# AIM-Harvard/pyradiomics

Hardware: AMD Instinct MI355X
Metric: Mvoxels/s for GLCM+GLRLM build, 512^3 vol @32 bins (higher is better)
Workload: dtype u8 levels / u32 counts / f64 out; 1 GPU; GLCM+GLRLM matrix build, 512^3 int32+uint8 volume resident in HBM, 32 grey levels, full mask, 13 angles, uniform levels; one volume per GPU (batch sharding, no collective); size=512, levels=32, dist=uniform, deferred_mode=pipeline

## Files before the change

### pyradiomics_amd/csrc/kernels_sweep.h

```cpp
#pragma once
#include "prad_runtime.h"

namespace prad {

typedef unsigned int u32;
typedef unsigned long long u64;

__global__ void __launch_bounds__(256) pack_levels_kernel(const int *__restrict__ image,
                                                          const uint8_t *__restrict__ mask, long long n, int NX,
                                                          int pitch, int padw, int Ng,
                                                          uint8_t *__restrict__ levels, int *__restrict__ flags,
                                                          int vec_ok, int shift, uint8_t *__restrict__ rowzero = nullptr) {
  const long long tid = (long long)blockIdx.x * blockDim.x + threadIdx.x;
  const long long nthreads = (long long)gridDim.x * blockDim.x;
  const bool linear = (padw == 0 && pitch == NX);
  int bad = 0;
  long long done = 0;
  if (vec_ok) {
    const long long n16 = n >> 4;
    const int upr = NX >> 4;
    const int4 *im4 = reinterpret_cast<const int4 *>(image);
    const uint4 *mk4 = reinterpret_cast<const uint4 *>(mask);
    for (long long t = tid; t < n16; t += nthreads) {
      const uint4 m = mk4[t];
// ... 323 lines not shown
__device__ __forceinline__ bool steps_break_group(W (&w)[LPL], const unsigned (&v)[U], const int (&sb)[U],
                                                  const bool (&uw)[U], int lane4) {
  bool m = false;
#pragma unroll
  for (int k = 0; k < U; k++) {
#pragma unroll
    for (int j = 0; j < LPL; j++) {
      const bool brk = uw[k] || (sb[k] == lane4 + j);
      m |= w[j].template step_brk<CHECK>((int)((v[k] >> (8 * j)) & 0xffu), brk);
    }
  }
  return m;
}
template <bool DO_GLCM, bool DO_GLRLM, bool FUSED>
__device__ __forceinline__ void flush_block_hist(const u32 *lds, const HistLayout &h, int Nr, int slot,
                                                 u32 *__restrict__ glcm_acc, u32 *__restrict__ glrlm_acc) {
  __syncthreads();
  const int Ng = h.Ng;
  if (FUSED) {
    const int Q = Ng + 1, P = (h.RS + 1) * Q;
    u32 *gd = glcm_acc + (size_t)slot * Ng * Ng;
    for (int i = threadIdx.x; i < Ng * Ng; i += blockDim.x) {
      const int p = i / Ng, c = i - p * Ng;
      if (p == c) continue;
      u32 v = 0;
      for (int l = 0; l <= h.RS; l++) v += lds[(p + 1) * P + l * Q + c + 1];
      if (v) atomicAdd(gd + i, v);
    }
    u32 *rd = glrlm_acc + (size_t)slot * Ng * Nr;
    for (int i = threadIdx.x; i < Ng * h.RS; i += blockDim.x) {
      const int p = i / h.RS, l = i - p * h.RS;
      u32 v = 0;
      for (int c = 0; c <= Ng; c++) v += lds[(p + 1) * P + l * Q + c];
      if (v) atomicAdd(rd + (size_t)p * Nr + l, v);
    }
    for (int i = threadIdx.x; i < Ng * h.RL; i += blockDim.x) {
      const int p = i / h.RL, l = h.RS + (i - p * h.RL);
      const u32 v = lds[h.g0 + i];
      if (v && l < Nr) atomicAdd(rd + (size_t)p * Nr + l, v);
    }
    return;
  }
  if (DO_GLCM) {
    u32 *dst = glcm_acc + (size_t)slot * Ng * Ng;
    for (int i = threadIdx.x; i < Ng * Ng; i += blockDim.x) {
      const u32 v = lds[i];
      if (v) atomicAdd(dst + i, v);
    }
  }
  if (DO_GLRLM) {
    const u32 *hr = lds + h.glrlm0;
    u32 *dst = glrlm_acc + (size_t)slot * Ng * Nr;
    for (int i = threadIdx.x; i < h.RS * Ng; i += blockDim.x) {
      const u32 v = hr[i];
      if (v) atomicAdd(dst + (size_t)(i % Ng) * Nr + (i / Ng), v);
// ... 279 lines not shown
    pairs += (unsigned long long)r * v;
    found |= (r > 0 && v != 0);
  }
  const u32 *grow = glcm_acc + ((size_t)a * Ng + i) * Ng;
  for (int j = lane; j < Ng; j += 64) found |= (grow[j] != 0);
  for (int o = 32; o > 0; o >>= 1) pairs += __shfl_xor(pairs, o);
  if (lane == 0) glcm_out[((size_t)i * Ng + i) * Na + a] = (double)pairs;
  if (__ballot(found) != 0 && lane == 0) multi[a] = 1;
}

struct AngleSet {
  int count;
  int off[PRAD_MAX_SWEEP][3];
};
template <typename T>
__global__ void __launch_bounds__(256) multi_check_kernel(AngleSet A, const T *__restrict__ L, int Nz, int Ny,
                                                          int Nx, int pitch, int *__restrict__ multi) {
  const int a = blockIdx.y;
  if (multi[a]) return;
  const int dz = A.off[a][0], dy = A.off[a][1], dx = A.off[a][2];
  const long long n = (long long)Nz * Ny * Nx, plane = (long long)Ny * Nx;
  const long long stride = (long long)gridDim.x * blockDim.x;
  for (long long i = (long long)blockIdx.x * blockDim.x + threadIdx.x; i < n; i += stride) {
    int z = (int)(i / plane);
    const int r = (int)(i - (long long)z * plane);
    int y = r / Nx, x = r - y * Nx;
    const int pz = z - dz, py = y - dy, px = x - dx;
    if ((unsigned)pz < (unsigned)Nz && (unsigned)py < (unsigned)Ny && (unsigned)px < (unsigned)Nx) continue;
    int cnt = 0;
    while ((unsigned)z < (unsigned)Nz && (unsigned)y < (unsigned)Ny && (unsigned)x < (unsigned)Nx) {
      cnt += L[((long long)z * Ny + y) * pitch + x] != 0;
      if (cnt > 1) {
        multi[a] = 1;
        return;
      }
      z += dz; y += dy; x += dx;
    }
  }
}

__global__ void finalize_glcm_kernel(const u32 *__restrict__ acc, const u32 *__restrict__ glrlm_acc, int Ng, int Nr,
                                     int Na, int diag_from_runs, double *__restrict__ out) {
  const long long idx = (long long)blockIdx.x * blockDim.x + threadIdx.x;
  const long long total = (long long)Ng * Ng * Na;
  if (idx >= total) return;
  const int a = (int)(idx % Na);
  const long long ij = idx / Na;
  const int i = (int)(ij / Ng), j = (int)(ij - (long long)i * Ng);
  if (diag_from_runs && i == j) return;
  out[idx] = (double)acc[(size_t)a * Ng * Ng + ij];
}

__global__ void __launch_bounds__(256) finalize_glcm_diag_kernel(const u32 *__restrict__ glcm_acc, u32 *glrlm_acc, int Ng, int Nr,
// ... 57 lines not shown
```

### pyradiomics_amd/csrc/kernels_sweepfw.h

```cpp
#pragma once
#include "kernels_sweep.h"

namespace prad {

enum FwPhase { FP_INIT, FP_GRAB, FP_CTRL, FP_ISSUE, FP_WAIT_ROWS, FP_WAIT_PACK, FP_GROUP, FP_PACK, FP_SLOW, FP_FLUSH, FP_DRAIN,
               FP_TOTAL, FP_REALTIME, FP_NGROUP, FP_NGROUP_PACK, FP_NSLOW, FP_COUNT };
#ifdef PRAD_FW_STAMPS
__device__ unsigned long long prad_fw_stamps[2 * 8192 * FP_COUNT];
struct FwClock {
  unsigned long long last, first, rt0;
  unsigned acc[FP_COUNT];
  __device__ __forceinline__ void start() {
#pragma unroll
    for (int i = 0; i < FP_COUNT; i++) acc[i] = 0;
    rt0 = __builtin_amdgcn_s_memrealtime();
    first = last = __builtin_readcyclecounter();
  }
  template <int PH>
  __device__ __forceinline__ void lap() {
    const unsigned long long now = __builtin_readcyclecounter();
    acc[PH] += (unsigned)(now - last);
    last = now;
  }
  template <int PH>
// ... 779 lines not shown
    asm volatile("" : "+v"(z));
    asm volatile(PRAD_FW_RCOL(0) PRAD_FW_RCOL(1) PRAD_FW_RCOL(2) PRAD_FW_RCOL(3)
                 : [s] "+v"(s), [t] "=&v"(t)
                 : [c] "v"(c), [x] "v"(x), [one] "v"(one), [P4] "s"(T.P4), [Q] "s"(T.Q), [z] "v"(z)
                 : "vcc", "memory");
  } else {
    asm volatile(PRAD_FW_RCOL_NZ(0) PRAD_FW_RCOL_NZ(1) PRAD_FW_RCOL_NZ(2) PRAD_FW_RCOL_NZ(3)
                 : [s] "+v"(s), [t] "=&v"(t)
                 : [c] "v"(c), [x] "v"(x), [one] "v"(one), [P4] "s"(T.P4), [Q] "s"(T.Q)
                 : "vcc", "memory");
  }
#undef PRAD_FW_RCOL
#undef PRAD_FW_RCOL_NZ
}

template <bool LONG, bool ZA>
__device__ __forceinline__ void fw_rows_role(const HistLayout &h, const FwTab &T, u32 *lds, const uint8_t *__restrict__ L,
                                             long long nrows, int NX, int pitch, int bx, int nblocks) {
  const int lane = threadIdx.x & 63, wave = threadIdx.x >> 6, wpb = blockDim.x >> 6;
  const int dummy = T.dummy0b + 4 * lane;
  u32 one = 1;
  asm volatile("" : "+v"(one));
  uint8_t *tile = reinterpret_cast<uint8_t *>(lds) + ((fw_lds_bytes(h) + 15) & ~(size_t)15) + (size_t)wave * 64 * PRAD_ROW_PITCH;
  const int RSTEP = nrows >= 4096 ? 8 : 1;
  const long long ngroups = RSTEP == 8 ? ((nrows + 511) / 512) * 8 : (nrows + 63) / 64;
  const long long nwaves = (long long)nblocks * wpb;
  const bool vec16 = (pitch & 15) == 0 && ((uintptr_t)L & 15) == 0;
  for (long long grp = (long long)bx * wpb + wave; grp < ngroups; grp += nwaves) {
    const long long r0 = RSTEP == 8 ? (grp >> 3) * 512 + (grp & 7) : grp * 64;
    int s = 0;
    u32 pw = 0;
    uint4 nx4[4];
    auto fetch = [&](int xc) __attribute__((always_inline)) {
#pragma unroll
      for (int j = 0; j < 4; j++) {
        const int rr = j * 16 + (lane >> 2);
        const int cx = xc + (lane & 3) * 16;
        uint4 q = make_uint4(0, 0, 0, 0);
        if (r0 + RSTEP * rr < nrows && cx < NX) {
          q = *reinterpret_cast<const uint4 *>(L + (r0 + RSTEP * rr) * pitch + cx);
          const int valid = NX - cx;
          if (valid < 16) {
            u32 *qw = reinterpret_cast<u32 *>(&q);
#pragma unroll
            for (int wd = 0; wd < 4; wd++) {
              const int keep = valid - 4 * wd;
// ... 14 lines not shown
      } else {
        const bool xin = xc + lane < NX;
#pragma unroll 8
        for (int rr = 0; rr < 64; rr++) {
          uint8_t b = 0;
          if (xin && r0 + RSTEP * rr < nrows) b = L[(r0 + RSTEP * rr) * pitch + xc + lane];
          tile[rr * PRAD_ROW_PITCH + lane] = b;
        }
      }
      __builtin_amdgcn_wave_barrier();
      const uint4 *row = reinterpret_cast<const uint4 *>(tile + lane * PRAD_ROW_PITCH);
#pragma unroll
      for (int q = 0; q < 4; q++) {
        const uint4 d = row[q];
        const u32 wds[4] = {d.x, d.y, d.z, d.w};
        const unsigned m = (pw >> 24) ? (unsigned)(s - __mul24((int)(pw >> 24), T.P4)) : 0u;
        if (LONG && __ballot(m + 16 * T.Q > (unsigned)T.lenlim) != 0) {
#pragma unroll 1
          for (int k = 0; k < 4; k++) {
            const u32 c = wds[k], x = __builtin_amdgcn_alignbyte(c, pw, 3);
            const unsigned m4 = (pw >> 24) ? (unsigned)(s - __mul24((int)(pw >> 24), T.P4)) : 0u;
            if (__ballot(m4 + 4 * T.Q > (unsigned)T.lenlim) != 0) {
#pragma unroll
              for (int b = 0; b < 4; b++) fw_checked<LONG>(T, dummy, s, (int)((x >> (8 * b)) & 0xffu), (int)((c >> (8 * b)) & 0xffu), false);
            } else {
              fw_row_word<ZA>(T, one, s, c, x);
            }
            pw = c;
          }
        } else {
#pragma unroll
          for (int k = 0; k < 4; k++) {
            fw_row_word<ZA>(T, one, s, wds[k], __builtin_amdgcn_alignbyte(wds[k], pw, 3));
            pw = wds[k];
          }
        }
      }
      __builtin_amdgcn_wave_barrier();
    }
    fw_checked<LONG>(T, dummy, s, (int)(pw >> 24), 0, false);
  }
}

template <bool LONG>
__global__ void __launch_bounds__(1024) sweep_fw_rows_kernel(const uint8_t *__restrict__ L, long long nrows, int NX, int pitch,
                                                            int slot, int Ng, int Nr, int RS, u32 *__restrict__ glcm_acc,
                                                            u32 *__restrict__ glrlm_acc, int *__restrict__ flags) {
  extern __shared__ u32 lds[];
  if (flags[0]) return;
  const HistLayout h = hist_layout(true, true, true, Ng, RS);
  if ((unsigned)(size_t)((lds_u32 *)lds) != 0u) {
    if (threadIdx.x == 0) atomicExch(flags + 2, 1);
    return;
  }
  for (int i = threadIdx.x; i < h.words + Ng + 1; i += blockDim.x) lds[i] = 0;
  __syncthreads();
  FwTab T;
  T.init(h, Nr, glrlm_acc + (size_t)slot * Ng * Nr);
  if (flags[3] != 0) fw_rows_role<LONG, true>(h, T, lds, L, nrows, NX, pitch, (int)blockIdx.x, (int)gridDim.x);
  else fw_rows_role<LONG, false>(h, T, lds, L, nrows, NX, pitch, (int)blockIdx.x, (int)gridDim.x);
  flush_block_hist<true, true, true>(lds + Ng + 1, h, Nr, slot, glcm_acc, glrlm_acc);
}

template <bool LONG, int K, bool HASPAD, bool PACK>
__global__ void __launch_bounds__(1024) sweep_fw_kernel(FwSet set, PackJob pj, const uint8_t *__restrict__ L,
                                                        const uint8_t *__restrict__ rowzero, int Ng, int Nr, int RS,
                                                        u32 *__restrict__ glcm_acc, u32 *__restrict__ glrlm_acc,
                                                        int *__restrict__ work, int *__restrict__ flags) {
  extern __shared__ u32 lds[];
  int role = 0;
  while (role + 1 < set.count && (int)blockIdx.x >= set.first_block[role + 1]) role++;
  const int bx = (int)blockIdx.x - set.first_block[role], nblocks = set.first_block[role + 1] - set.first_block[role];
  const int wpb = (int)(blockDim.x >> 6);
  const long long pw = __builtin_amdgcn_readfirstlane((int)(blockIdx.x * wpb + (threadIdx.x >> 6)));
  PackWave pk(pj, pw, (long long)gridDim.x * wpb);
  FwClock clk;
  clk.start();
#ifdef PRAD_FW_SETPRIO
  __builtin_amdgcn_s_setprio(PRAD_FW_SETPRIO);
#endif
  if (flags[0] == 0) {
    const bool anyzero = flags[3] != 0;
    const HistLayout h = hist_layout(true, true, true, Ng, RS);
// ... 6 lines not shown
      const FwDesc &D = set.d[role];
      FwTab T;
      T.init(h, Nr, glrlm_acc + (size_t)D.slot * Ng * Nr);
      int *wk = work + PRAD_FW_WORK_STRIDE * PRAD_FW_DOMAINS * role;
      if (D.dx == 0) {
        FwWave<LONG, K, 0, HASPAD, PACK> w(T, set.NX);
        w.run(D, set.NX, set.pitch, set.nrows, L, rowzero, anyzero, wk, bx, nblocks, pk, pj, set.xcd != 0, clk);
      } else if (D.dx > 0) {
        FwWave<LONG, K, 1, HASPAD, PACK> w(T, set.NX);
        w.run(D, set.NX, set.pitch, set.nrows, L, rowzero, anyzero, wk, bx, nblocks, pk, pj, set.xcd != 0, clk);
      } else {
        FwWave<LONG, K, -1, HASPAD, PACK> w(T, set.NX);
        w.run(D, set.NX, set.pitch, set.nrows, L, rowzero, anyzero, wk, bx, nblocks, pk, pj, set.xcd != 0, clk);
      }
      clk.lap<FP_CTRL>();
      flush_block_hist<true, true, true>(lds + Ng + 1, h, Nr, D.slot, glcm_acc, glrlm_acc);
      clk.lap<FP_FLUSH>();
    }
  }
  if (PACK) pk.drain(pj);
  clk.lap<FP_DRAIN>();
  clk.store(PACK ? 1 : 0);
}

}
```

### pyradiomics_amd/csrc/prad_api.hip

```cpp
#include "prad_runtime.h"
#include "kernels_generic.h"
#include "kernels_pairs.h"
#include "kernels_sweep.h"
#include "kernels_sweepfw.h"
#include "kernels_sweepfw2.h"
#include "kernels_neigh.h"
#include "kernels_glszm.h"
#include "kernels_voxel.h"
#include "kernels_voxslide.h"
#include "kernels_mcc.h"
#include "kernels_voxtex.h"
#include "kernels_binning.h"

#include <algorithm>
#include <atomic>
#include <chrono>
#include <cmath>
#include <condition_variable>
#include <cstdlib>
#include <deque>
#include <limits>
#include <mutex>
#include <thread>

// ... 529 lines not shown

template <bool G, bool R, bool LNG, bool F>
int launch_lines(Call &k, const SweepPlan &p, const uint8_t *levels, int Ng, int Nr, u32 *glcm_acc, u32 *glrlm_acc,
                 int *multi) {
  if (p.LPL == 4) return launch_lines_lpl<G, R, LNG, F, 4>(k, p, levels, Ng, Nr, glcm_acc, glrlm_acc, multi);
  if (p.LPL == 2) return launch_lines_lpl<G, R, LNG, F, 2>(k, p, levels, Ng, Nr, glcm_acc, glrlm_acc, multi);
  return launch_lines_lpl<G, R, LNG, F, 1>(k, p, levels, Ng, Nr, glcm_acc, glrlm_acc, multi);
}

template <bool LNG, int K, bool HASPAD, bool PACK>
int launch_fw_kpp(Call &k, const SweepPlan &p, const PackJob &pj, const uint8_t *levels, const uint8_t *rowzero, int Ng, int Nr,
                  u32 *glcm_acc, u32 *glrlm_acc, int *multi, int *flags_d) {
  PRAD_HIP(hipFuncSetAttribute(reinterpret_cast<const void *>(&sweep_fw_kernel<LNG, K, HASPAD, PACK>),
                               hipFuncAttributeMaxDynamicSharedMemorySize, (int)p.lds_fw));
  hipLaunchKernelGGL((sweep_fw_kernel<LNG, K, HASPAD, PACK>), dim3(p.fw_blocks), dim3(p.fw_threads), p.lds_fw, k.s, p.fwset, pj,
                     levels, rowzero, Ng, Nr, p.RSfw, glcm_acc, glrlm_acc, multi + 2 * PRAD_MAX_SWEEP + PRAD_FW_WORK_STRIDE, flags_d);
  return check_launch("sweep_fw_kernel");
}
template <bool LNG, int K, bool HASPAD>
int launch_fw_kp(Call &k, const SweepPlan &p, const PackJob &pj, const uint8_t *levels, const uint8_t *rowzero, int Ng, int Nr,
                 u32 *glcm_acc, u32 *glrlm_acc, int *multi, int *flags_d) {
  if (pj.n16 > 0) return launch_fw_kpp<LNG, K, HASPAD, true>(k, p, pj, levels, rowzero, Ng, Nr, glcm_acc, glrlm_acc, multi, flags_d);
  return launch_fw_kpp<LNG, K, HASPAD, false>(k, p, pj, levels, rowzero, Ng, Nr, glcm_acc, glrlm_acc, multi, flags_d);
}
template <bool LNG, int K>
int launch_fw_k(Call &k, const SweepPlan &p, const PackJob &pj, const uint8_t *levels, const uint8_t *rowzero, int Ng, int Nr,
                u32 *glcm_acc, u32 *glrlm_acc, int *multi, int *flags_d) {
  if (p.Nx != 64 * K) return launch_fw_kp<LNG, K, true>(k, p, pj, levels, rowzero, Ng, Nr, glcm_acc, glrlm_acc, multi, flags_d);
  return launch_fw_kp<LNG, K, false>(k, p, pj, levels, rowzero, Ng, Nr, glcm_acc, glrlm_acc, multi, flags_d);
}
int launch_fw(Call &k, const SweepPlan &p, const PackJob &pj, const uint8_t *levels, const uint8_t *rowzero, int Ng, int Nr,
// ... 29 lines not shown
  if (p.Nx != 64 * K)
    return p.skip1 ? launch_fw2_khs<LNG, K, true, true>(k, p, pj, levels16, Ng, Nr, glcm_acc, glrlm_acc, work, flags_d)
                   : launch_fw2_khs<LNG, K, true, false>(k, p, pj, levels16, Ng, Nr, glcm_acc, glrlm_acc, work, flags_d);
  return p.skip1 ? launch_fw2_khs<LNG, K, false, true>(k, p, pj, levels16, Ng, Nr, glcm_acc, glrlm_acc, work, flags_d)
                 : launch_fw2_khs<LNG, K, false, false>(k, p, pj, levels16, Ng, Nr, glcm_acc, glrlm_acc, work, flags_d);
}
int launch_fw2(Call &k, const SweepPlan &p, const PackJob &pj, const uint8_t *levels16, int Ng, int Nr, u32 *glcm_acc, u32 *glrlm_acc,
               int *multi, int *flags_d) {
  if (p.LONGfw2) return p.fwK == 4 ? launch_fw2_k<true, 4>(k, p, pj, levels16, Ng, Nr, glcm_acc, glrlm_acc, multi, flags_d)
                                 : launch_fw2_k<true, 8>(k, p, pj, levels16, Ng, Nr, glcm_acc, glrlm_acc, multi, flags_d);
  return p.fwK == 4 ? launch_fw2_k<false, 4>(k, p, pj, levels16, Ng, Nr, glcm_acc, glrlm_acc, multi, flags_d)
                    : launch_fw2_k<false, 8>(k, p, pj, levels16, Ng, Nr, glcm_acc, glrlm_acc, multi, flags_d);
}

template <bool LNG>
int launch_fw_rows(Call &k, const SweepPlan &p, const uint8_t *levels, int Ng, int Nr, u32 *glcm_acc, u32 *glrlm_acc, int *flags_d) {
  const long long nrows = (long long)p.Nz * p.Ny, groups = nrows >= 4096 ? ((nrows + 511) / 512) * 8 : (nrows + 63) / 64;
  const int wpb = p.fw_rows_threads / 64;
  const unsigned gx = (unsigned)std::max<long long>(1, std::min<long long>((groups + wpb - 1) / wpb, (long long)cu_count()));
  PRAD_HIP(hipFuncSetAttribute(reinterpret_cast<const void *>(&sweep_fw_rows_kernel<LNG>),
                               hipFuncAttributeMaxDynamicSharedMemorySize, (int)p.lds_fw_rows));
  hipLaunchKernelGGL((sweep_fw_rows_kernel<LNG>), dim3(gx), dim3(p.fw_rows_threads), p.lds_fw_rows, k.s, levels, nrows, p.Nx,
                     p.pitch, p.row_slot, Ng, Nr, p.RSfw_rows, glcm_acc, glrlm_acc, flags_d);
  return check_launch("sweep_fw_rows_kernel");
}

template <bool LNG>
int launch_fw2_rows(Call &k, const SweepPlan &p, const uint8_t *levels16, int Ng, int Nr, u32 *glcm_acc, u32 *glrlm_acc, int *flags_d) {
  const long long nrows = (long long)p.Nz * p.Ny, groups = nrows >= 4096 ? ((nrows + 511) / 512) * 8 : (nrows + 63) / 64;
  const int wpb = p.fw2r_waves;
  const unsigned gx = (unsigned)std::max<long long>(1, std::min<long long>((groups + wpb - 1) / wpb, (long long)cu_count()));
  PRAD_HIP(hipFuncSetAttribute(reinterpret_cast<const void *>(&sweep_fw2_rows_kernel<LNG>),
                               hipFuncAttributeMaxDynamicSharedMemorySize, (int)p.lds_fw2_rows));
  hipLaunchKernelGGL((sweep_fw2_rows_kernel<LNG>), dim3(gx), dim3(64 * wpb), p.lds_fw2_rows, k.s, levels16, nrows, p.Nx, p.pitch16,
                     p.row_slot, Ng, Nr, p.RS2r, p.fw2r_copies, glcm_acc, glrlm_acc, flags_d);
  return check_launch("sweep_fw2_rows_kernel");
}

// ... 22 lines not shown
  for (size_t i = t; i < nc; i += nt) c3[i] = 0;
}

struct VolState {
  bool valid = false;
  SweepPlan p;
  int Ng = 0, Nr = 0, Na = 0;
  double *glcm = nullptr, *glrlm = nullptr;
  uint8_t *levels = nullptr, *rowzero = nullptr;
  uint8_t *levels16 = nullptr;
  u32 *acc = nullptr, *glcm_acc = nullptr, *glrlm_acc = nullptr;
  int *multi = nullptr;
  int *flags_d = nullptr;
  bool packed_inline = false;
  int lane = -1;
};

bool fin_side() {
  static const bool on = getenv("PRAD_FINALIZE_STREAM") != nullptr && atoi(getenv("PRAD_FINALIZE_STREAM")) != 0;
  return on;
}
int fin_wait_for_lane(hipStream_t s, int lane);

int vol_prepare(Call &k, const SweepPlan &p, int Ng, int Nr, double *glcm, double *glrlm, VolState &v) {
  Context &c = *k.c;
  if (fin_side() && c.lane >= 0) PRAD_TRY(fin_wait_for_lane(k.s, c.lane));
  v.lane = c.lane;
  v.valid = true;
  v.p = p;
  v.Ng = Ng;
  v.Nr = Nr;
  v.Na = k.Na;
  v.glcm = glcm;
  v.glrlm = glrlm;
  v.flags_d = k.flags_d;
  const long long nrows = (long long)p.Nz * p.Ny;
  v.levels = nullptr;
// ... 3 lines not shown
  }
  v.levels16 = nullptr;
  if (p.fw2) {
    PRAD_TRY(c.get<uint8_t>("levels16", (size_t)nrows * p.pitch16 + 4096, &v.levels16));
    v.levels16 += 2048;
  }
  const size_t nglcm = glcm ? (size_t)k.Na * Ng * Ng : 0, nglrlm = glrlm ? (size_t)k.Na * Ng * Nr : 0;
  const size_t nctl = 2 * PRAD_MAX_SWEEP + (size_t)PRAD_FW_WORK_STRIDE * (PRAD_FW_DOMAINS * PRAD_MAX_SWEEP + 1);
  PRAD_TRY(c.get<u32>("sweep_acc", nglcm + nglrlm + nctl, &v.acc));
  v.glcm_acc = v.acc;
  v.glrlm_acc = v.acc + nglcm;
  v.multi = (int *)(v.acc + nglcm + nglrlm);
  v.rowzero = nullptr;
  if (p.fw) PRAD_TRY(c.get<uint8_t>("rowzero", (size_t)nrows + 64, &v.rowzero));
  const size_t acc_w = nglcm + nglrlm + nctl, rz_w = v.rowzero ? ((size_t)nrows + 3) / 4 : 0;
  const size_t total_w = acc_w + rz_w + 4;
  const unsigned gx = (unsigned)std::max<size_t>(1, std::min<size_t>((total_w / 4 + 255) / 256, 1024));
  hipLaunchKernelGGL(zero3_kernel, dim3(gx), dim3(256), 0, k.s, v.acc, acc_w, reinterpret_cast<u32 *>(v.rowzero), rz_w,
                     reinterpret_cast<u32 *>(v.flags_d), (size_t)4);
  return check_launch("zero3_kernel");
}

bool pipeline_volume(const SweepPlan &p, bool glcm, bool glrlm) {
  if (!(p.ok && p.lines.count > 0 && glcm && glrlm)) return false;
  return (p.fw && p.fused) || (p.fw2 && !getenv("PRAD_FW2_LANES"));
}
bool pack_inline_ok(const Call &k, const VolState &v) {
  if (!(v.glcm && v.glrlm && v.p.pitch == v.p.Nx && v.p.padw == 0 && (k.g.n % 16) == 0 &&
        ((((uintptr_t)k.image) | ((uintptr_t)k.mask) | ((uintptr_t)v.levels)) & 15) == 0))
    return false;
// ... 37 lines not shown
                       v.levels16, v.levels, v.flags_d);
    return check_launch("pack_levels16_kernel");
  }
  const int vec_ok = p.vec_rows && ((((uintptr_t)k.image) | ((uintptr_t)k.mask) | ((uintptr_t)v.levels)) & 15) == 0;
  const unsigned gx = (unsigned)std::max<long long>(1, std::min<long long>((k.g.n / 16 + 255) / 256, 4096));
  const int shift = (v.glcm && v.glrlm && p.fused) ? PRAD_FUSED_SHIFT : 0;
  hipLaunchKernelGGL(pack_levels_kernel, dim3(gx), dim3(256), 0, k.s, k.image, k.mask, k.g.n, p.Nx, p.pitch, p.padw,
                     v.Ng, v.levels, v.flags_d, vec_ok, shift, v.rowzero);
  return check_launch("pack_levels_kernel");
}

template <bool G, bool R, bool F>
int launch_sweeps(Call &k, const VolState &v, const PackJob &pj) {
  const SweepPlan &p = v.p;
  if (p.lines.count > 0 && p.fw && G && R && F) {
    static const bool rows_side = getenv("PRAD_ROWS_STREAM") != nullptr;
    if (rows_side && p.row_slot >= 0) {
      static thread_local hipStream_t side = nullptr;
      static thread_local hipEvent_t e0 = nullptr, e1 = nullptr;
      if (!side) {
        int lo = 0, hi = 0;
        PRAD_HIP(hipDeviceGetStreamPriorityRange(&lo, &hi));
        PRAD_HIP(hipStreamCreateWithPriority(&side, hipStreamNonBlocking, getenv("PRAD_ROWS_STREAM_PRIO") ? atoi(getenv("PRAD_ROWS_STREAM_PRIO")) : lo));
        PRAD_HIP(hipEventCreateWithFlags(&e0, hipEventDisableTiming));
        PRAD_HIP(hipEventCreateWithFlags(&e1, hipEventDisableTiming));
      }
      PRAD_HIP(hipEventRecord(e0, k.s));
      PRAD_HIP(hipStreamWaitEvent(side, e0, 0));
      {
        Timed t(*k.c, "sweep", k.s);
        PRAD_TRY(launch_fw(k, p, pj, v.levels, v.rowzero, v.Ng, v.Nr, v.glcm_acc, v.glrlm_acc, v.multi, v.flags_d));
      }
      Call k2 = k;
      k2.s = side;
      if (p.RSfw_rows < v.Nr) PRAD_TRY(launch_fw_rows<true>(k2, p, v.levels, v.Ng, v.Nr, v.glcm_acc, v.glrlm_acc, v.flags_d));
      else PRAD_TRY(launch_fw_rows<false>(k2, p, v.levels, v.Ng, v.Nr, v.glcm_acc, v.glrlm_acc, v.flags_d));
      PRAD_HIP(hipEventRecord(e1, side));
      PRAD_HIP(hipStreamWaitEvent(k.s, e1, 0));
      return PRAD_OK;
    }
    {
      Timed t(*k.c, "sweep", k.s);
      PRAD_TRY(launch_fw(k, p, pj, v.levels, v.rowzero, v.Ng, v.Nr, v.glcm_acc, v.glrlm_acc, v.multi, v.flags_d));
    }
    if (p.row_slot >= 0) {
      Timed t(*k.c, "rows", k.s);
      if (p.RSfw_rows < v.Nr) PRAD_TRY(launch_fw_rows<true>(k, p, v.levels, v.Ng, v.Nr, v.glcm_acc, v.glrlm_acc, v.flags_d));
      else PRAD_TRY(launch_fw_rows<false>(k, p, v.levels, v.Ng, v.Nr, v.glcm_acc, v.glrlm_acc, v.flags_d));
    }
    return PRAD_OK;
  }
  if (p.fw2 && G && R && !F && p.lines.count > 0) {
    {
      Timed t(*k.c, "sweep", k.s);
      PRAD_TRY(launch_fw2(k, p, pj, v.levels16, v.Ng, v.Nr, v.glcm_acc, v.glrlm_acc, v.multi, v.flags_d));
    }
    if (p.row_slot >= 0) {
      Timed t(*k.c, "rows", k.s);
      if (p.fw2_rows) {
        if (p.LONGfw2r) PRAD_TRY(launch_fw2_rows<true>(k, p, v.levels16, v.Ng, v.Nr, v.glcm_acc, v.glrlm_acc, v.flags_d));
        else PRAD_TRY(launch_fw2_rows<false>(k, p, v.levels16, v.Ng, v.Nr, v.glcm_acc, v.glrlm_acc, v.flags_d));
      } else if (p.LONGr) {
        PRAD_TRY((launch_rows<G, R, true, F>(k, p, v.levels, v.Ng, v.Nr, v.glcm_acc, v.glrlm_acc, v.multi)));
// ... 29 lines not shown
__global__ void latch_flags_kernel(const int *__restrict__ flags, int *__restrict__ sticky) {
  if (flags[0] || flags[2]) sticky[0] = 1;
}

__global__ void latch_any_flag_kernel(const int *__restrict__ flags, int *__restrict__ sticky) {
  if (flags[0] || flags[1] || flags[2]) sticky[0] = 1;
}
int latch_neigh(Context &c, Call &k) {
  int *sticky = nullptr;
  PRAD_TRY(c.get<int>("deferred_sticky", 16, &sticky));
  hipLaunchKernelGGL(latch_any_flag_kernel, dim3(1), dim3(1), 0, k.s, (const int *)k.flags_d, sticky);
  return check_launch("latch_any_flag_kernel");
}

int vol_finalize(Call &k, const VolState &v, int *sticky) {
  Context &c = *k.c;
  const SweepPlan &p = v.p;
  const int Ng = v.Ng, Nr = v.Nr, Na = v.Na;
  double *glcm = v.glcm, *glrlm = v.glrlm;
  bool latched = false;
  {
    Timed t(c, "finalize", k.s);
    const bool runs_diag = p.fused || p.fw2;
    if (p.fw2 && p.skip1 && p.lines.count > 0 && !(glcm && glrlm && p.row_slot >= 0))
      return fail(PRAD_E_UNSUPPORTED, "sweep plan derives runs of length 1 but the call cannot restore them");
    if (glcm && glrlm && runs_diag) {
      const int nb1 = (int)blocks_for((long long)Ng * Ng * Na), nb2 = (Ng * Na + 3) / 4;
      hipLaunchKernelGGL(finalize_glcm_diag_kernel, dim3(nb1 + nb2), dim3(256), 0, k.s, v.glcm_acc, v.glrlm_acc, Ng, Nr, Na, nb1,
                         glcm, v.multi, (p.fw2 && p.skip1 && p.lines.count > 0) ? p.row_slot : -1);
      PRAD_TRY(check_launch("finalize_glcm_diag_kernel"));
// ... 25 lines not shown
  }
  if (sticky && !latched) {
    hipLaunchKernelGGL(latch_flags_kernel, dim3(1), dim3(1), 0, k.s, v.flags_d, sticky);
    PRAD_TRY(check_launch("latch_flags_kernel"));
  }
  return PRAD_OK;
}

int sweep_glcm_glrlm(Call &k, const SweepPlan &p, int Ng, int Nr, double *glcm, double *glrlm, bool *used) {
  Context &c = *k.c;
  VolState v;
  PRAD_TRY(vol_prepare(k, p, Ng, Nr, glcm, glrlm, v));
  PRAD_TRY(vol_pack_standalone(k, v));
  PackJob pj;
  memset(&pj, 0, sizeof(pj));
  PRAD_TRY(vol_sweep(k, v, pj));
  int *sticky = nullptr;
  if (c.deferred) PRAD_TRY(c.get<int>("deferred_sticky", 16, &sticky));
  PRAD_TRY(vol_finalize(k, v, sticky));
  if (c.deferred) {
    *used = true;
    return PRAD_OK;
  }
  PRAD_TRY(read_flags(k));
  *used = (k.flags_h[0] == 0 && k.flags_h[2] == 0);
  return PRAD_OK;
}

struct PipeState {
  VolState pending;
  hipStream_t s = nullptr;
  unsigned long long seq = 0;
  hipEvent_t ev = nullptr;
  int mode = -1;
  hipStream_t fin = nullptr;
  hipEvent_t fin_in = nullptr, fin_all = nullptr, fin_done[4] = {};
  bool fin_used[4] = {};
};
PipeState &pipe_state() {
  static thread_local PipeState p;
// ... 11 lines not shown

int pipeline_retire(Context &c, hipStream_t s, const PackJob &pj) {
  PipeState &ps = pipe_state();
  if (ps.s != s) {
    if (!ps.ev) PRAD_HIP(hipEventCreateWithFlags(&ps.ev, hipEventDisableTiming));
    PRAD_HIP(hipEventRecord(ps.ev, ps.s));
    PRAD_HIP(hipStreamWaitEvent(s, ps.ev, 0));
  }
  Call k;
  k.c = &c;
  k.s = s;
  k.Na = ps.pending.Na;
  k.flags_d = ps.pending.flags_d;
  int *sticky = nullptr;
  PRAD_TRY(pipeline_sticky(c, &sticky));
  PRAD_TRY(vol_sweep(k, ps.pending, pj));
  if (fin_side() && ps.pending.lane >= 0 && ps.pending.lane < 4) {
    if (!ps.fin) {
      PRAD_HIP(hipStreamCreateWithFlags(&ps.fin, hipStreamNonBlocking));
      PRAD_HIP(hipEventCreateWithFlags(&ps.fin_in, hipEventDisableTiming));
      PRAD_HIP(hipEventCreateWithFlags(&ps.fin_all, hipEventDisableTiming));
      for (int l = 0; l < 4; l++) PRAD_HIP(hipEventCreateWithFlags(&ps.fin_done[l], hipEventDisableTiming));
    }
    PRAD_HIP(hipEventRecord(ps.fin_in, s));
    PRAD_HIP(hipStreamWaitEvent(ps.fin, ps.fin_in, 0));
    Call k2 = k;
    k2.s = ps.fin;
    PRAD_TRY(vol_finalize(k2, ps.pending, sticky));
    PRAD_HIP(hipEventRecord(ps.fin_done[ps.pending.lane], ps.fin));
    ps.fin_used[ps.pending.lane] = true;
// ... 747 lines not shown
  for (const auto &kv : ctx().bufs) total += (long long)kv.second.cap;
  return total;
}
namespace {
void release_image_queues();
}
int prad_release_workspace(void) {
  Context &c = ctx();
  if (pipe_state().pending.valid) {
    (void)pipeline_flush(c);
    if (pipe_state().s) (void)hipStreamSynchronize(pipe_state().s);
    (void)fin_join(nullptr, true);
    pipe_state().pending.valid = false;
  }
  glszm_state().valid = false;
  for (auto &kv : c.bufs) {
    if (kv.second.p) (void)hipFree(kv.second.p);
    kv.second.p = nullptr;
    kv.second.cap = 0;
  }
  (void)hipDeviceSynchronize();
  for (auto &kv : c.pinned) {
    if (kv.second.p) (void)hipHostFree(kv.second.p);
    kv.second.p = nullptr;
    kv.second.cap = 0;
  }
  c.bufs.clear();
  c.pinned.clear();
  if (c.arena) (void)hipHostFree(c.arena);
  c.arena = nullptr;
// ... 754 lines not shown
```

### pyradiomics_amd/csrc/prad_runtime.h

```cpp
#pragma once

#include <hip/hip_runtime.h>
#include <stdint.h>
#include <stdio.h>
#include <stdarg.h>
#include <string.h>
#include <stdlib.h>
#include <string>
#include <vector>
#include <map>

#include "../../include/pyradiomics_amd.h"

namespace prad {

struct ErrorState {
  char msg[512];
  ErrorState() { msg[0] = 0; }
};
inline ErrorState &err_state() {
  static thread_local ErrorState e;
  return e;
}
inline int fail(int code, const char *fmt, ...) {
// ... 3 lines not shown
  va_end(ap);
  return code;
}

#define PRAD_HIP(call)                                                                              \
  do {                                                                                              \
    hipError_t e_ = (call);                                                                         \
    if (e_ != hipSuccess)                                                                           \
      return ::prad::fail(e_ == hipErrorOutOfMemory ? PRAD_E_NOMEM : PRAD_E_HIP, "%s failed: %s (%s:%d)", \
                          #call, hipGetErrorString(e_), __FILE__, __LINE__);                        \
  } while (0)

struct DevBuf {
  void *p = nullptr;
  size_t cap = 0;
};

struct KernelTime {
  std::string family;
  hipEvent_t a, b;
};

#define PRAD_MAX_LANES 4
#define PRAD_ARENA_BYTES (4u << 20)

struct Context {
  int device = 0;
  bool device_set = false;
  hipStream_t own_stream = nullptr;
  std::map<std::string, DevBuf> bufs;
// ... 68 lines not shown
    for (int l = 0; l < PRAD_MAX_LANES; l++)
      if (lane_stream[l]) {
        PRAD_HIP(hipEventRecord(lane_in[l], lane_stream[l]));
        PRAD_HIP(hipStreamWaitEvent(s, lane_in[l], 0));
      }
    return PRAD_OK;
  }
  int lanes_sync() {
    for (int l = 0; l < PRAD_MAX_LANES; l++)
      if (lane_stream[l]) PRAD_HIP(hipStreamSynchronize(lane_stream[l]));
    return PRAD_OK;
  }

  int get(const char *name, size_t bytes, void **out) {
    DevBuf &b = bufs[key(name)];
    if (b.cap < bytes) {
      if (b.p) (void)hipFree(b.p);
      b.p = nullptr;
      b.cap = 0;
      size_t want = bytes + bytes / 8 + 256;
      hipError_t e = hipMalloc(&b.p, want);
      if (e != hipSuccess) {
        b.p = nullptr;
        return fail(PRAD_E_NOMEM, "hipMalloc(%zu) for workspace '%s' failed: %s", want, name, hipGetErrorString(e));
      }
      b.cap = want;
    }
    *out = b.p;
    return PRAD_OK;
  }
// ... 206 lines not shown
```

Before: 285,800 Mvoxels/s.

## Fuse finalize, multi-check and workspace zeroing into rows sweep kernel epilogue

```diff
diff --git a/pyradiomics_amd/csrc/kernels_sweep.h b/pyradiomics_amd/csrc/kernels_sweep.h
--- a/pyradiomics_amd/csrc/kernels_sweep.h
+++ b/pyradiomics_amd/csrc/kernels_sweep.h
@@ -361,31 +361,43 @@
 }
 template <bool DO_GLCM, bool DO_GLRLM, bool FUSED>
 __device__ __forceinline__ void flush_block_hist(const u32 *lds, const HistLayout &h, int Nr, int slot,
-                                                 u32 *__restrict__ glcm_acc, u32 *__restrict__ glrlm_acc) {
+                                                 u32 *__restrict__ glcm_acc, u32 *__restrict__ glrlm_acc,
+                                                 int *multi = nullptr) {
   __syncthreads();
   const int Ng = h.Ng;
   if (FUSED) {
     const int Q = Ng + 1, P = (h.RS + 1) * Q;
+    bool found = false;
     u32 *gd = glcm_acc + (size_t)slot * Ng * Ng;
     for (int i = threadIdx.x; i < Ng * Ng; i += blockDim.x) {
       const int p = i / Ng, c = i - p * Ng;
       if (p == c) continue;
       u32 v = 0;
       for (int l = 0; l <= h.RS; l++) v += lds[(p + 1) * P + l * Q + c + 1];
-      if (v) atomicAdd(gd + i, v);
+      if (v) {
+        atomicAdd(gd + i, v);
+        found = true;
+      }
     }
     u32 *rd = glrlm_acc + (size_t)slot * Ng * Nr;
     for (int i = threadIdx.x; i < Ng * h.RS; i += blockDim.x) {
       const int p = i / h.RS, l = i - p * h.RS;
       u32 v = 0;
       for (int c = 0; c <= Ng; c++) v += lds[(p + 1) * P + l * Q + c];
-      if (v) atomicAdd(rd + (size_t)p * Nr + l, v);
+      if (v) {
+        atomicAdd(rd + (size_t)p * Nr + l, v);
+        found |= l > 0;
+      }
     }
     for (int i = threadIdx.x; i < Ng * h.RL; i += blockDim.x) {
       const int p = i / h.RL, l = h.RS + (i - p * h.RL);
       const u32 v = lds[h.g0 + i];
-      if (v && l < Nr) atomicAdd(rd + (size_t)p * Nr + l, v);
-    }
+      if (v && l < Nr) {
+        atomicAdd(rd + (size_t)p * Nr + l, v);
+        found = true;
+      }
+    }
+    if (multi && __ballot(found) != 0 && (threadIdx.x & 63) == 0) multi[slot] = 1;
     return;
   }
   if (DO_GLCM) {
@@ -695,14 +707,11 @@
   int off[PRAD_MAX_SWEEP][3];
 };
 template <typename T>
-__global__ void __launch_bounds__(256) multi_check_kernel(AngleSet A, const T *__restrict__ L, int Nz, int Ny,
-                                                          int Nx, int pitch, int *__restrict__ multi) {
-  const int a = blockIdx.y;
-  if (multi[a]) return;
+__device__ __forceinline__ void multi_check_angle(const AngleSet &A, int a, const T *__restrict__ L, int Nz, int Ny, int Nx,
+                                                  int pitch, int *flag, long long first, long long stride) {
   const int dz = A.off[a][0], dy = A.off[a][1], dx = A.off[a][2];
   const long long n = (long long)Nz * Ny * Nx, plane = (long long)Ny * Nx;
-  const long long stride = (long long)gridDim.x * blockDim.x;
-  for (long long i = (long long)blockIdx.x * blockDim.x + threadIdx.x; i < n; i += stride) {
+  for (long long i = first; i < n; i += stride) {
     int z = (int)(i / plane);
     const int r = (int)(i - (long long)z * plane);
     int y = r / Nx, x = r - y * Nx;
@@ -712,12 +721,54 @@
     while ((unsigned)z < (unsigned)Nz && (unsigned)y < (unsigned)Ny && (unsigned)x < (unsigned)Nx) {
       cnt += L[((long long)z * Ny + y) * pitch + x] != 0;
       if (cnt > 1) {
-        multi[a] = 1;
+        __hip_atomic_store(flag, 1, __ATOMIC_RELAXED, __HIP_MEMORY_SCOPE_AGENT);
         return;
       }
       z += dz; y += dy; x += dx;
     }
   }
+}
+template <typename T>
+__global__ void __launch_bounds__(256) multi_check_kernel(AngleSet A, const T *__restrict__ L, int Nz, int Ny,
+                                                          int Nx, int pitch, int *__restrict__ multi) {
+  const int a = blockIdx.y;
+  if (multi[a]) return;
+  multi_check_angle<T>(A, a, L, Nz, Ny, Nx, pitch, multi + a, (long long)blockIdx.x * blockDim.x + threadIdx.x,
+                       (long long)gridDim.x * blockDim.x);
+}
+
+template <int U>
+__device__ __forceinline__ void finalize_fused_row(u32 *__restrict__ glcm_acc, u32 *__restrict__ glrlm_acc, int Ng, int Nr, int Na, int a,
+                                                   int i, int col0, double *__restrict__ glcm_out, double *__restrict__ glrlm_out,
+                                                   int g, int T) {
+  u32 *__restrict__ row = glrlm_acc + ((size_t)a * Ng + i) * Nr;
+  u32 *__restrict__ grow = glcm_acc + ((size_t)a * Ng + i) * Ng;
+  unsigned long long pairs = 0;
+  for (int r0 = 0; r0 < Nr; r0 += T * U) {
+    u32 v[U];
+#pragma unroll
+    for (int k = 0; k < U; k++) {
+      const int r = r0 + T * k + g;
+      v[k] = r < Nr ? row[r] : 0u;
+    }
+#pragma unroll
+    for (int k = 0; k < U; k++) {
+      const int r = r0 + T * k + g;
+      if (r >= Nr) continue;
+      pairs += (unsigned long long)r * v[k];
+      if (r > 0 || col0 >= 0) {
+        glrlm_out[((size_t)i * Nr + r) * Na + a] = (r == 0 && col0 == 0) ? 0.0 : (double)v[k];
+        row[r] = 0;
+      }
+    }
+  }
+  for (int j = g; j < Ng; j += T) {
+    const u32 gv = grow[j];
+    if (j != i) glcm_out[((size_t)i * Ng + j) * Na + a] = (double)gv;
+    grow[j] = 0;
+  }
+  for (int o = T >> 1; o > 0; o >>= 1) pairs += __shfl_xor(pairs, o);
+  if (g == 0) glcm_out[((size_t)i * Ng + i) * Na + a] = (double)pairs;
 }
 
 __global__ void finalize_glcm_kernel(const u32 *__restrict__ acc, const u32 *__restrict__ glrlm_acc, int Ng, int Nr,
diff --git a/pyradiomics_amd/csrc/kernels_sweepfw.h b/pyradiomics_amd/csrc/kernels_sweepfw.h
--- a/pyradiomics_amd/csrc/kernels_sweepfw.h
+++ b/pyradiomics_amd/csrc/kernels_sweepfw.h
@@ -817,9 +817,14 @@
 #undef PRAD_FW_RCOL_NZ
 }
 
-template <bool LONG, bool ZA>
-__device__ __forceinline__ void fw_rows_role(const HistLayout &h, const FwTab &T, u32 *lds, const uint8_t *__restrict__ L,
+__device__ __forceinline__ int fw_masked_bytes(u32 w) {
+  return __popc((((w >> 2) & 0x3f3f3f3fu) + 0x3f3f3f3fu) & 0x40404040u);
+}
+
+template <bool LONG, bool ZA, bool XM = false>
+__device__ __forceinline__ bool fw_rows_role(const HistLayout &h, const FwTab &T, u32 *lds, const uint8_t *__restrict__ L,
                                              long long nrows, int NX, int pitch, int bx, int nblocks) {
+  bool xm = false;
   const int lane = threadIdx.x & 63, wave = threadIdx.x >> 6, wpb = blockDim.x >> 6;
   const int dummy = T.dummy0b + 4 * lane;
   u32 one = 1;
@@ -833,6 +838,7 @@
     const long long r0 = RSTEP == 8 ? (grp >> 3) * 512 + (grp & 7) : grp * 64;
     int s = 0;
     u32 pw = 0;
+    int nmask = 0;
     uint4 nx4[4];
     auto fetch = [&](int xc) __attribute__((always_inline)) {
 #pragma unroll
@@ -877,6 +883,7 @@
       for (int q = 0; q < 4; q++) {
         const uint4 d = row[q];
         const u32 wds[4] = {d.x, d.y, d.z, d.w};
+        if (XM) nmask += fw_masked_bytes(d.x) + fw_masked_bytes(d.y) + fw_masked_bytes(d.z) + fw_masked_bytes(d.w);
         const unsigned m = (pw >> 24) ? (unsigned)(s - __mul24((int)(pw >> 24), T.P4)) : 0u;
         if (LONG && __ballot(m + 16 * T.Q > (unsigned)T.lenlim) != 0) {
 #pragma unroll 1
@@ -902,34 +909,126 @@
       __builtin_amdgcn_wave_barrier();
     }
     fw_checked<LONG>(T, dummy, s, (int)(pw >> 24), 0, false);
-  }
-}
-
-template <bool LONG>
+    if (XM) xm |= nmask >= 2;
+  }
+  return xm;
+}
+
+struct RowsEpi {
+  double *glcm_out, *glrlm_out;
+  int *multi;
+  int nctl;
+  u32 *rowzero;
+  long long nrz;
+  int *sticky;
+  int *flags_out;
+  int Na, Nz, Ny;
+  AngleSet aset;
+};
+
+__device__ __forceinline__ void rows_epilogue_lines(const RowsEpi &e, const uint8_t *__restrict__ L, int NX, int pitch, int slot,
+                                                    int Ng, int Nr, u32 *glcm_acc, u32 *glrlm_acc, const int *flags) {
+  const int lane = threadIdx.x & 63, wave = threadIdx.x >> 6, wpb = (int)(blockDim.x >> 6);
+  const int nb = (int)gridDim.x, bx = (int)blockIdx.x;
+  int *mx = e.multi + PRAD_MAX_SWEEP;
+  for (int u = wave * nb + bx; u < (e.Na - 1) * Ng; u += nb * wpb) {
+    int a = u / Ng;
+    const int i = u - a * Ng;
+    a += a >= slot ? 1 : 0;
+    finalize_fused_row<8>(glcm_acc, glrlm_acc, Ng, Nr, e.Na, a, i, e.multi[a] ? 1 : -1, e.glcm_out, e.glrlm_out, lane, 64);
+  }
+  for (long long w = (long long)bx * blockDim.x + threadIdx.x; w < e.nrz; w += (long long)nb * blockDim.x) e.rowzero[w] = 0;
+  if (flags[0] == 0)
+    for (int a = 0; a < e.Na; a++)
+      if (a != slot && !e.multi[a] && !__hip_atomic_load(mx + a, __ATOMIC_RELAXED, __HIP_MEMORY_SCOPE_AGENT))
+        multi_check_angle<uint8_t>(e.aset, a, L, e.Nz, e.Ny, NX, pitch, mx + a, (long long)bx * blockDim.x + threadIdx.x,
+                                   (long long)nb * blockDim.x);
+}
+
+__device__ __forceinline__ void rows_epilogue(const RowsEpi &e, u32 *lds, int slot, int Ng, int Nr, u32 *glcm_acc, u32 *glrlm_acc,
+                                              int *flags, bool xm) {
+  const int lane = threadIdx.x & 63;
+  const int nb = (int)gridDim.x;
+  int *mx = e.multi + PRAD_MAX_SWEEP;
+  if (__ballot(xm) != 0 && lane == 0) atomicOr(mx + slot, 1);
+  asm volatile("s_waitcnt vmcnt(0)" ::: "memory");
+  __syncthreads();
+  if (threadIdx.x == 0) {
+    __builtin_amdgcn_fence(__ATOMIC_RELEASE, "agent");
+    asm volatile("s_waitcnt vmcnt(0)" ::: "memory");
+    const int last = __hip_atomic_fetch_add(e.multi + 2 * PRAD_MAX_SWEEP, 1, __ATOMIC_RELAXED, __HIP_MEMORY_SCOPE_AGENT) == nb - 1;
+    if (last) {
+      __builtin_amdgcn_fence(__ATOMIC_ACQUIRE, "agent");
+      asm volatile("s_waitcnt vmcnt(0)" ::: "memory");
+    }
+    lds[0] = (u32)last;
+  }
+  __syncthreads();
+  if (lds[0] == 0) return;
+  const int f0 = __hip_atomic_load(flags + 0, __ATOMIC_RELAXED, __HIP_MEMORY_SCOPE_AGENT);
+  const int f1 = __hip_atomic_load(flags + 1, __ATOMIC_RELAXED, __HIP_MEMORY_SCOPE_AGENT);
+  const int f2 = __hip_atomic_load(flags + 2, __ATOMIC_RELAXED, __HIP_MEMORY_SCOPE_AGENT);
+  const int f3 = __hip_atomic_load(flags + 3, __ATOMIC_RELAXED, __HIP_MEMORY_SCOPE_AGENT);
+  const bool xmulti = f3 == 0 || __hip_atomic_load(mx + slot, __ATOMIC_RELAXED, __HIP_MEMORY_SCOPE_AGENT) != 0;
+  {
+    int T = 64;
+    while (T > 1 && Ng * T > (int)blockDim.x) T >>= 1;
+    for (int i = threadIdx.x / T; i < Ng; i += blockDim.x / T)
+      finalize_fused_row<32>(glcm_acc, glrlm_acc, Ng, Nr, e.Na, slot, i, xmulti ? 1 : 0, e.glcm_out, e.glrlm_out, threadIdx.x & (T - 1), T);
+  }
+  for (int u = threadIdx.x; u < e.Na * Ng; u += blockDim.x) {
+    const int a = u / Ng, i = u - a * Ng;
+    if (a == slot || e.multi[a]) continue;
+    u32 *w = glrlm_acc + ((size_t)a * Ng + i) * Nr;
+    e.glrlm_out[(size_t)i * Nr * e.Na + a] = __hip_atomic_load(mx + a, __ATOMIC_RELAXED, __HIP_MEMORY_SCOPE_AGENT) ? (double)*w : 0.0;
+    *w = 0;
+  }
+  __syncthreads();
+  if (threadIdx.x == 0) {
+    if (e.sticky && (f0 || f2)) e.sticky[0] = 1;
+    if (e.flags_out) {
+      e.flags_out[0] = f0;
+      e.flags_out[1] = f1;
+      e.flags_out[2] = f2;
+      e.flags_out[3] = f3;
+    }
+  }
+  if (threadIdx.x < 4) flags[threadIdx.x] = 0;
+  for (int w = threadIdx.x; w < e.nctl; w += blockDim.x) e.multi[w] = 0;
+}
+
+template <bool LONG, bool EPI>
 __global__ void __launch_bounds__(1024) sweep_fw_rows_kernel(const uint8_t *__restrict__ L, long long nrows, int NX, int pitch,
                                                             int slot, int Ng, int Nr, int RS, u32 *__restrict__ glcm_acc,
-                                                            u32 *__restrict__ glrlm_acc, int *__restrict__ flags) {
+                                                            u32 *__restrict__ glrlm_acc, int *__restrict__ flags, RowsEpi e) {
   extern __shared__ u32 lds[];
-  if (flags[0]) return;
-  const HistLayout h = hist_layout(true, true, true, Ng, RS);
-  if ((unsigned)(size_t)((lds_u32 *)lds) != 0u) {
-    if (threadIdx.x == 0) atomicExch(flags + 2, 1);
-    return;
-  }
-  for (int i = threadIdx.x; i < h.words + Ng + 1; i += blockDim.x) lds[i] = 0;
-  __syncthreads();
-  FwTab T;
-  T.init(h, Nr, glrlm_acc + (size_t)slot * Ng * Nr);
-  if (flags[3] != 0) fw_rows_role<LONG, true>(h, T, lds, L, nrows, NX, pitch, (int)blockIdx.x, (int)gridDim.x);
-  else fw_rows_role<LONG, false>(h, T, lds, L, nrows, NX, pitch, (int)blockIdx.x, (int)gridDim.x);
-  flush_block_hist<true, true, true>(lds + Ng + 1, h, Nr, slot, glcm_acc, glrlm_acc);
+  bool xm = false;
+  if (EPI) rows_epilogue_lines(e, L, NX, pitch, slot, Ng, Nr, glcm_acc, glrlm_acc, flags);
+  if (flags[0] == 0) {
+    const HistLayout h = hist_layout(true, true, true, Ng, RS);
+    if ((unsigned)(size_t)((lds_u32 *)lds) != 0u) {
+      if (threadIdx.x == 0) atomicExch(flags + 2, 1);
+    } else {
+      for (int i = threadIdx.x; i < h.words + Ng + 1; i += blockDim.x) lds[i] = 0;
+      __syncthreads();
+      FwTab T;
+      T.init(h, Nr, glrlm_acc + (size_t)slot * Ng * Nr);
+      if (flags[3] != 0) xm = fw_rows_role<LONG, true, EPI>(h, T, lds, L, nrows, NX, pitch, (int)blockIdx.x, (int)gridDim.x);
+      else fw_rows_role<LONG, false>(h, T, lds, L, nrows, NX, pitch, (int)blockIdx.x, (int)gridDim.x);
+      flush_block_hist<true, true, true>(lds + Ng + 1, h, Nr, slot, glcm_acc, glrlm_acc);
+    }
+  }
+  if (EPI) {
+    __syncthreads();
+    rows_epilogue(e, lds, slot, Ng, Nr, glcm_acc, glrlm_acc, flags, xm);
+  }
 }
 
 template <bool LONG, int K, bool HASPAD, bool PACK>
 __global__ void __launch_bounds__(1024) sweep_fw_kernel(FwSet set, PackJob pj, const uint8_t *__restrict__ L,
                                                         const uint8_t *__restrict__ rowzero, int Ng, int Nr, int RS,
                                                         u32 *__restrict__ glcm_acc, u32 *__restrict__ glrlm_acc,
-                                                        int *__restrict__ work, int *__restrict__ flags) {
+                                                        int *__restrict__ work, int *__restrict__ flags, int *__restrict__ multi) {
   extern __shared__ u32 lds[];
   int role = 0;
   while (role + 1 < set.count && (int)blockIdx.x >= set.first_block[role + 1]) role++;
@@ -966,7 +1065,7 @@
         w.run(D, set.NX, set.pitch, set.nrows, L, rowzero, anyzero, wk, bx, nblocks, pk, pj, set.xcd != 0, clk);
       }
       clk.lap<FP_CTRL>();
-      flush_block_hist<true, true, true>(lds + Ng + 1, h, Nr, D.slot, glcm_acc, glrlm_acc);
+      flush_block_hist<true, true, true>(lds + Ng + 1, h, Nr, D.slot, glcm_acc, glrlm_acc, multi);
       clk.lap<FP_FLUSH>();
     }
   }
diff --git a/pyradiomics_amd/csrc/prad_api.hip b/pyradiomics_amd/csrc/prad_api.hip
--- a/pyradiomics_amd/csrc/prad_api.hip
+++ b/pyradiomics_amd/csrc/prad_api.hip
@@ -567,7 +567,8 @@
   PRAD_HIP(hipFuncSetAttribute(reinterpret_cast<const void *>(&sweep_fw_kernel<LNG, K, HASPAD, PACK>),
                                hipFuncAttributeMaxDynamicSharedMemorySize, (int)p.lds_fw));
   hipLaunchKernelGGL((sweep_fw_kernel<LNG, K, HASPAD, PACK>), dim3(p.fw_blocks), dim3(p.fw_threads), p.lds_fw, k.s, p.fwset, pj,
-                     levels, rowzero, Ng, Nr, p.RSfw, glcm_acc, glrlm_acc, multi + 2 * PRAD_MAX_SWEEP + PRAD_FW_WORK_STRIDE, flags_d);
+                     levels, rowzero, Ng, Nr, p.RSfw, glcm_acc, glrlm_acc, multi + 2 * PRAD_MAX_SWEEP + PRAD_FW_WORK_STRIDE, flags_d,
+                     multi);
   return check_launch("sweep_fw_kernel");
 }
 template <bool LNG, int K, bool HASPAD>
@@ -627,14 +628,24 @@
 }
 
 template <bool LNG>
-int launch_fw_rows(Call &k, const SweepPlan &p, const uint8_t *levels, int Ng, int Nr, u32 *glcm_acc, u32 *glrlm_acc, int *flags_d) {
+int launch_fw_rows(Call &k, const SweepPlan &p, const uint8_t *levels, int Ng, int Nr, u32 *glcm_acc, u32 *glrlm_acc, int *flags_d,
+                   const RowsEpi *epi = nullptr) {
   const long long nrows = (long long)p.Nz * p.Ny, groups = nrows >= 4096 ? ((nrows + 511) / 512) * 8 : (nrows + 63) / 64;
   const int wpb = p.fw_rows_threads / 64;
   const unsigned gx = (unsigned)std::max<long long>(1, std::min<long long>((groups + wpb - 1) / wpb, (long long)cu_count()));
-  PRAD_HIP(hipFuncSetAttribute(reinterpret_cast<const void *>(&sweep_fw_rows_kernel<LNG>),
+  if (epi) {
+    PRAD_HIP(hipFuncSetAttribute(reinterpret_cast<const void *>(&sweep_fw_rows_kernel<LNG, true>),
+                                 hipFuncAttributeMaxDynamicSharedMemorySize, (int)p.lds_fw_rows));
+    hipLaunchKernelGGL((sweep_fw_rows_kernel<LNG, true>), dim3(gx), dim3(p.fw_rows_threads), p.lds_fw_rows, k.s, levels, nrows, p.Nx,
+                       p.pitch, p.row_slot, Ng, Nr, p.RSfw_rows, glcm_acc, glrlm_acc, flags_d, *epi);
+    return check_launch("sweep_fw_rows_kernel");
+  }
+  RowsEpi none;
+  memset(&none, 0, sizeof(none));
+  PRAD_HIP(hipFuncSetAttribute(reinterpret_cast<const void *>(&sweep_fw_rows_kernel<LNG, false>),
                                hipFuncAttributeMaxDynamicSharedMemorySize, (int)p.lds_fw_rows));
-  hipLaunchKernelGGL((sweep_fw_rows_kernel<LNG>), dim3(gx), dim3(p.fw_rows_threads), p.lds_fw_rows, k.s, levels, nrows, p.Nx,
-                     p.pitch, p.row_slot, Ng, Nr, p.RSfw_rows, glcm_acc, glrlm_acc, flags_d);
+  hipLaunchKernelGGL((sweep_fw_rows_kernel<LNG, false>), dim3(gx), dim3(p.fw_rows_threads), p.lds_fw_rows, k.s, levels, nrows, p.Nx,
+                     p.pitch, p.row_slot, Ng, Nr, p.RSfw_rows, glcm_acc, glrlm_acc, flags_d, none);
   return check_launch("sweep_fw_rows_kernel");
 }
 
@@ -687,13 +698,60 @@
   int *flags_d = nullptr;
   bool packed_inline = false;
   int lane = -1;
+  bool epi = false;
+  int *sticky = nullptr;
+  int *flags_out = nullptr;
+  size_t acc_w = 0, rz_w = 0;
+  std::string ws_acc, ws_rz, ws_flags;
 };
 
 bool fin_side() {
   static const bool on = getenv("PRAD_FINALIZE_STREAM") != nullptr && atoi(getenv("PRAD_FINALIZE_STREAM")) != 0;
   return on;
 }
+bool rows_side() {
+  static const bool on = getenv("PRAD_ROWS_STREAM") != nullptr;
+  return on;
+}
 int fin_wait_for_lane(hipStream_t s, int lane);
+
+bool rows_epilogue_volume(const SweepPlan &p, bool glcm, bool glrlm) {
+  static const bool off = getenv("PRAD_NO_ROWS_EPILOGUE") != nullptr;
+  return !off && glcm && glrlm && p.fw && p.fused && p.lines.count > 0 && p.row_slot >= 0 && !fin_side() && !rows_side();
+}
+
+struct WsClean {
+  bool valid = false;
+  u32 *acc = nullptr;
+  uint8_t *rowzero = nullptr;
+  int *flags = nullptr;
+  size_t acc_w = 0, rz_w = 0;
+  unsigned long long g_acc = 0, g_rz = 0, g_flags = 0;
+};
+std::map<std::string, WsClean> &ws_clean() {
+  static thread_local std::map<std::string, WsClean> m;
+  return m;
+}
+unsigned long long buf_gets(Context &c, const std::string &key) {
+  auto it = c.bufs.find(key);
+  return it == c.bufs.end() ? 0 : it->second.gets;
+}
+void ws_mark_clean(Context &c, const VolState &v) {
+  WsClean &w = ws_clean()[v.ws_acc];
+  w.valid = true;
+  w.acc = v.acc;
+  w.rowzero = v.rowzero;
+  w.flags = v.flags_d;
+  w.acc_w = v.acc_w;
+  w.rz_w = v.rz_w;
+  w.g_acc = buf_gets(c, v.ws_acc);
+  w.g_rz = buf_gets(c, v.ws_rz);
+  w.g_flags = buf_gets(c, v.ws_flags);
+}
+void ws_mark_dirty(const VolState &v) {
+  auto it = ws_clean().find(v.ws_acc);
+  if (it != ws_clean().end()) it->second.valid = false;
+}
 
 int vol_prepare(Call &k, const SweepPlan &p, int Ng, int Nr, double *glcm, double *glrlm, VolState &v) {
   Context &c = *k.c;
@@ -727,6 +785,20 @@
   v.rowzero = nullptr;
   if (p.fw) PRAD_TRY(c.get<uint8_t>("rowzero", (size_t)nrows + 64, &v.rowzero));
   const size_t acc_w = nglcm + nglrlm + nctl, rz_w = v.rowzero ? ((size_t)nrows + 3) / 4 : 0;
+  v.epi = rows_epilogue_volume(p, glcm != nullptr, glrlm != nullptr);
+  v.acc_w = acc_w;
+  v.rz_w = rz_w;
+  v.ws_acc = c.key("sweep_acc");
+  v.ws_rz = c.key("rowzero");
+  v.ws_flags = c.key("flags");
+  {
+    WsClean &w = ws_clean()[v.ws_acc];
+    const bool clean = w.valid && v.rowzero && w.acc == v.acc && w.acc_w == acc_w && w.rowzero == v.rowzero && w.rz_w == rz_w &&
+                       w.flags == v.flags_d && buf_gets(c, v.ws_acc) == w.g_acc + 1 && buf_gets(c, v.ws_rz) == w.g_rz + 1 &&
+                       buf_gets(c, v.ws_flags) == w.g_flags + 1;
+    w.valid = false;
+    if (clean) return PRAD_OK;
+  }
   const size_t total_w = acc_w + rz_w + 4;
   const unsigned gx = (unsigned)std::max<size_t>(1, std::min<size_t>((total_w / 4 + 255) / 256, 1024));
   hipLaunchKernelGGL(zero3_kernel, dim3(gx), dim3(256), 0, k.s, v.acc, acc_w, reinterpret_cast<u32 *>(v.rowzero), rz_w,
@@ -794,8 +866,7 @@
 int launch_sweeps(Call &k, const VolState &v, const PackJob &pj) {
   const SweepPlan &p = v.p;
   if (p.lines.count > 0 && p.fw && G && R && F) {
-    static const bool rows_side = getenv("PRAD_ROWS_STREAM") != nullptr;
-    if (rows_side && p.row_slot >= 0) {
+    if (rows_side() && p.row_slot >= 0) {
       static thread_local hipStream_t side = nullptr;
       static thread_local hipEvent_t e0 = nullptr, e1 = nullptr;
       if (!side) {
@@ -824,9 +895,26 @@
       PRAD_TRY(launch_fw(k, p, pj, v.levels, v.rowzero, v.Ng, v.Nr, v.glcm_acc, v.glrlm_acc, v.multi, v.flags_d));
     }
     if (p.row_slot >= 0) {
+      RowsEpi e;
+      memset(&e, 0, sizeof(e));
+      if (v.epi) {
+        e.glcm_out = v.glcm;
+        e.glrlm_out = v.glrlm;
+        e.multi = v.multi;
+        e.nctl = (int)(v.acc_w - (size_t)(v.multi - (int *)v.acc));
+        e.rowzero = reinterpret_cast<u32 *>(v.rowzero);
+        e.nrz = (long long)v.rz_w;
+        e.sticky = v.sticky;
+        e.flags_out = v.flags_out;
+        e.Na = v.Na;
+        e.Nz = p.Nz;
+        e.Ny = p.Ny;
+        e.aset = p.aset;
+      }
       Timed t(*k.c, "rows", k.s);
-      if (p.RSfw_rows < v.Nr) PRAD_TRY(launch_fw_rows<true>(k, p, v.levels, v.Ng, v.Nr, v.glcm_acc, v.glrlm_acc, v.flags_d));
-      else PRAD_TRY(launch_fw_rows<false>(k, p, v.levels, v.Ng, v.Nr, v.glcm_acc, v.glrlm_acc, v.flags_d));
+      if (p.RSfw_rows < v.Nr) PRAD_TRY(launch_fw_rows<true>(k, p, v.levels, v.Ng, v.Nr, v.glcm_acc, v.glrlm_acc, v.flags_d, v.epi ? &e : nullptr));
+      else PRAD_TRY(launch_fw_rows<false>(k, p, v.levels, v.Ng, v.Nr, v.glcm_acc, v.glrlm_acc, v.flags_d, v.epi ? &e : nullptr));
+      if (v.epi) ws_mark_clean(*k.c, v);
     }
     return PRAD_OK;
   }
@@ -886,6 +974,7 @@
 }
 
 int vol_finalize(Call &k, const VolState &v, int *sticky) {
+  if (v.epi) return PRAD_OK;
   Context &c = *k.c;
   const SweepPlan &p = v.p;
   const int Ng = v.Ng, Nr = v.Nr, Na = v.Na;
@@ -941,16 +1030,20 @@
   PRAD_TRY(vol_pack_standalone(k, v));
   PackJob pj;
   memset(&pj, 0, sizeof(pj));
-  PRAD_TRY(vol_sweep(k, v, pj));
   int *sticky = nullptr;
   if (c.deferred) PRAD_TRY(c.get<int>("deferred_sticky", 16, &sticky));
+  v.sticky = sticky;
+  if (v.epi && !c.deferred) PRAD_TRY(c.get<int>("flags_out", 4, &v.flags_out));
+  PRAD_TRY(vol_sweep(k, v, pj));
   PRAD_TRY(vol_finalize(k, v, sticky));
   if (c.deferred) {
     *used = true;
     return PRAD_OK;
   }
-  PRAD_TRY(read_flags(k));
+  PRAD_HIP(hipMemcpyAsync(k.flags_h, v.flags_out ? v.flags_out : k.flags_d, sizeof(int) * 4, hipMemcpyDeviceToHost, k.s));
+  PRAD_HIP(hipStreamSynchronize(k.s));
   *used = (k.flags_h[0] == 0 && k.flags_h[2] == 0);
+  if (!*used) ws_mark_dirty(v);
   return PRAD_OK;
 }
 
@@ -992,6 +1085,7 @@
   k.flags_d = ps.pending.flags_d;
   int *sticky = nullptr;
   PRAD_TRY(pipeline_sticky(c, &sticky));
+  ps.pending.sticky = sticky;
   PRAD_TRY(vol_sweep(k, ps.pending, pj));
   if (fin_side() && ps.pending.lane >= 0 && ps.pending.lane < 4) {
     if (!ps.fin) {
@@ -1769,6 +1863,7 @@
     pipe_state().pending.valid = false;
   }
   glszm_state().valid = false;
+  ws_clean().clear();
   for (auto &kv : c.bufs) {
     if (kv.second.p) (void)hipFree(kv.second.p);
     kv.second.p = nullptr;
diff --git a/pyradiomics_amd/csrc/prad_runtime.h b/pyradiomics_amd/csrc/prad_runtime.h
--- a/pyradiomics_amd/csrc/prad_runtime.h
+++ b/pyradiomics_amd/csrc/prad_runtime.h
@@ -41,6 +41,7 @@
 struct DevBuf {
   void *p = nullptr;
   size_t cap = 0;
+  unsigned long long gets = 0;
 };
 
 struct KernelTime {
@@ -139,6 +140,7 @@
 
   int get(const char *name, size_t bytes, void **out) {
     DevBuf &b = bufs[key(name)];
+    b.gets++;
     if (b.cap < bytes) {
       if (b.p) (void)hipFree(b.p);
       b.p = nullptr;
```

Result: slower. 275,500 Mvoxels/s (-3.6%).
